# MisterBourbaki/vector-quantization-by-ml

Measured on AMD Instinct MI355X. Metric: vectors quantized/sec on [B*N,D]x[K,D] argmin; indices bit-exact vs CPU, higher is better.
Workload: dtype f32; 1 GPU; VectorQuantize dim=256 codebook_size=1024, batch [256,1024,256] per GPU, eval

## Files before the change

vector-quantization-by-ml_amd/csrc/vq_kernels.hip:

```cpp

#include <hip/hip_runtime.h>
#include <stdint.h>
#include <stdio.h>
#include <stdlib.h>
#include <string.h>

#include <initializer_list>
#include <type_traits>

#include "../../include/vq_mi355x.h"

#ifndef VQ_PART
#define VQ_PART -1
#endif
#define VQ_OWN(part) (VQ_PART < 0 || VQ_PART == (part))

typedef float f32x2 __attribute__((ext_vector_type(2)));
typedef float f32x4 __attribute__((ext_vector_type(4)));
typedef float f32x16 __attribute__((ext_vector_type(16)));

namespace {

#include "vq_common.inc"
#if VQ_OWN(0)
// ... 105 lines not shown
        return c;
    }
    static const bool no_persist = getenv("VQ_NO_PERSIST") != nullptr;
    const bool train = p.ste || p.loss_part;
    const int nsub = p.ntiles * sub_tiles(DP);
    if (whole_call && !no_persist && DP == 256 && waves == 8 && p.Q == 1 && !p.lse && !p.xt && p.vec_x && p.vec_fin && p.D % 4 == 0 &&
        (p.out || p.loss_part) &&
        !(train && getenv("VQ_NO_PERSIST_TRAIN") != nullptr) &&
        nsub >= kPersistMinSub && nsub <= kPersistMaxSub &&
        one_block_grid_x(p.M, waves) * H >= 2ll * cus) {
        c.kind = kPersist;
        c.train = train;
        c.screened = !train && metric == VQ_METRIC_EUCLID && !p.best && getenv("VQ_NO_SCREEN") == nullptr &&
                     (scr_cached ? screen_list_bytes(H, p.M) : screen_bytes(H, p.M, p.ntiles)) <= scr_room &&
                     scr_image_bytes(p.ntiles) < (1ll << 31) && (long long)H * p.M < (1ll << 31);
        c.cached = c.screened && scr_cached;
        return c;
    }
    if (DP == 512 && p.tiles_per_split >= 8 && use_pair512() &&
        (p.Q == 1 || (getenv("VQ_PAIR_NO_MULTI") == nullptr && p.Q <= PairGeo::max_stages()))) {
        c.kind = kPair;
        c.waves = 8;
    }
    return c;
}

template <int DP, int WAVES, int METRIC, int MULTI, bool LSE = false, int XT = 0, int WIDE = 0>
int launch_search_t(const SearchParams &p, int H, int splits, hipStream_t s) {
    using G = Geo<DP, WAVES>;
    const size_t lds = (size_t)(MULTI ? G::MAIN_FLOATS_M : G::MAIN_FLOATS_S) * 4 + (size_t)WAVES * p.Q * 32 * 4 +
                       ((MULTI && p.loss_part) ? (size_t)WAVES * p.Q * 64 * 4 : 0);
    if (lds > 160 * 1024) return fail(VQ_E_UNSUPPORTED, "vq_search: LDS budget exceeded (too many residual stages)");
    return launch<vq_search_mfma<DP, WAVES, METRIC, MULTI, LSE, XT, WIDE>, kBigLds>(
        dim3((unsigned)one_block_grid_x(p.M, WAVES), (unsigned)H, (unsigned)splits), dim3(WAVES * 64), lds, s, "vq_search_mfma launch", p);
}

template <int DP, int WAVES>
constexpr size_t multi_lds_bytes(int Q, bool with_loss) {
    return (size_t)Geo<DP, WAVES>::MAIN_FLOATS_M * 4 + (size_t)WAVES * Q * 32 * 4 + (with_loss ? (size_t)WAVES * Q * 64 * 4 : 0);
}

template <int DP, int WAVES>
int max_stages_t(bool with_loss) {
    int q = 1;
    while (q < 4096 && multi_lds_bytes<DP, WAVES>(q + 1, with_loss) <= 160 * 1024) ++q;
    return q;
}

template <int DP, int WAVES>
int launch_search_m(const SearchParams &p, int H, int splits, int metric, hipStream_t s) {
    return with_metric(metric, [&](auto m) {
        constexpr int ME = decltype(m)::value;
        if (p.Q > 1)
            return p.ste ? launch_search_t<DP, WAVES, ME, 2>(p, H, splits, s) : launch_search_t<DP, WAVES, ME, 1>(p, H, splits, s);
        if (p.xt == 1) return launch_search_t<DP, WAVES, ME, 0, false, 1>(p, H, splits, s);
        if (p.xt == 2) return launch_search_t<DP, WAVES, ME, 0, false, 2>(p, H, splits, s);
        if (p.lse) return launch_search_t<DP, WAVES, ME, 0, true>(p, H, splits, s);
        return launch_search_t<DP, WAVES, ME, 0>(p, H, splits, s);
    });
}

template <int METRIC, bool LSE = false, int XT = 0, int WIDE = 0, int MULTI = 0>
int launch_pair_t(const SearchParams &p, int H, int splits, hipStream_t s) {
    return launch<vq_search_pair512<METRIC, LSE, XT, WIDE, MULTI>, kBigLds>(dim3((unsigned)pair_grid_x(p.M), (unsigned)H, (unsigned)splits), dim3(512),
                                                                            PairGeo::lds_bytes(MULTI ? p.Q : 1), s, "vq_search_pair512 launch", p);
}

#if VQ_OWN(4)
int launch_pair_any(const SearchParams &p, int H, int splits, int metric, hipStream_t s) {
    return with_metric(metric, [&](auto m) {
        constexpr int ME = decltype(m)::value;
        if (p.Q > 1)
            return p.ste ? launch_pair_t<ME, false, 0, 0, 2>(p, H, splits, s) : launch_pair_t<ME, false, 0, 0, 1>(p, H, splits, s);
        if (p.xt == 1) return launch_pair_t<ME, false, 1>(p, H, splits, s);
        if (p.xt == 2) return launch_pair_t<ME, false, 2>(p, H, splits, s);
        if (p.lse) return launch_pair_t<ME, true>(p, H, splits, s);
        return launch_pair_t<ME>(p, H, splits, s);
    });
}
#endif

template <int DP>
int launch_pack_scr(const float *packed, long long pk_hs, int K, int ntiles, int H, char *img, long long img_hs, unsigned *ctrl, hipStream_t s) {
    return launch<vq_pack_scr_kernel<DP>>(dim3((unsigned)ntiles, (unsigned)H), dim3(256), 0, s, "vq_pack_scr launch", packed, pk_hs, K, ntiles, img,
                                           img_hs, ctrl);
}

template <int METRIC, bool TRAIN = false, bool SCREEN = false>
int launch_persist_t(const SearchParams &p, int H, int cus, hipStream_t s, bool scr_cached = false) {
    using G = Geo<256, 8>;
    const size_t lds = (size_t)G::MAIN_FLOATS_S * 4 + 2 * 8 * 32 * 4;
    if constexpr (SCREEN) {
        if (!scr_cached)
            if (int rc = launch_pack_scr<256>(p.packed, p.pk_hs, p.K, p.ntiles, H, (char *)p.scr, p.scr_hs, p.scr_count, s)) return rc;
    }
    if (int rc = launch<vq_search_persist<256, 8, METRIC, TRAIN, SCREEN>, kBigLds>(dim3((unsigned)persist_grid_x(p.M, H, cus), (unsigned)H, 1), dim3(512),
                                                                                   lds, s, "vq_search_persist launch", p))
        return rc;
    if constexpr (SCREEN) {
        const int flags = getenv("VQ_RESOLVE_NO_SPLIT") ? kResolveNoSplit : 0;
        return launch<vq_resolve_rows_kernel<256>, kBigLds>(dim3((unsigned)(cus > 0 ? cus : 1)), dim3(kResolveWaves * 64), resolve_lds_bytes<256>(), s,
                                                            "vq_resolve_rows launch", p, H, flags);
    }
    return 0;
}

template <int DP, int METRIC>
int launch_resident_t(const SearchParams &p, int H, int cus, hipStream_t s) {
    const size_t lds = ResGeo<DP>::lds_bytes(p.res_img_floats, p.res_nbuf);
    const long long nwb = (p.M + 31) / 32;
    long long gx = cus / H;
    if (gx < 1) gx = 1;
    if (gx > (nwb + 7) / 8) gx = (nwb + 7) / 8;
    auto go = [&](auto multibuf) {
        return launch<vq_search_resident<DP, METRIC, decltype(multibuf)::value>, kBigLds>(dim3((unsigned)gx, (unsigned)H, 1), dim3(512), lds, s,
                                                                                          "vq_search_resident launch", p);
    };
    if constexpr (DP < 128) {
        if (p.res_nbuf > 1) return go(std::true_type{});
    }
    return go(std::false_type{});
}

template <int DP>
int launch_resident_m(const SearchParams &p, int H, int cus, int metric, hipStream_t s) {
    return with_metric(metric, [&](auto m) { return launch_resident_t<DP, decltype(m)::value>(p, H, cus, s); });
}

template <int DP, int WAVES, int METRIC, int MODE>
int launch_aux_t(const AuxParams &p, int H, hipStream_t s) {
    return launch<vq_sweep_aux<DP, WAVES, METRIC, MODE>, kBigLds>(dim3((unsigned)one_block_grid_x(p.M, WAVES), (unsigned)H, 1), dim3(WAVES * 64),
                                                                  (size_t)Geo<DP, WAVES>::MAIN_FLOATS * 4, s, "vq_sweep_aux launch", p);
}

template <int DP, int WAVES>
int launch_aux_m(const AuxParams &p, int H, int metric, int mode, hipStream_t s) {
    return with_metric(metric, [&](auto m) {
        constexpr int ME = decltype(m)::value;
        return mode == kAuxSims ? launch_aux_t<DP, WAVES, ME, kAuxSims>(p, H, s) : launch_aux_t<DP, WAVES, ME, kAuxStats>(p, H, s);
    });
}

template <int DP, int METRIC>
int launch_ce_bwd_t(const CeBwdParams &p, int H, hipStream_t s) {
    const size_t stage_floats = (size_t)4 * (32 * CeGeo<DP>::GS + 96), main_floats = (size_t)Geo<DP, 4>::MAIN_FLOATS;
    return launch<vq_ce_backward<DP, METRIC>, kBigLds>(dim3((unsigned)((p.M + 127) / 128), (unsigned)H, (unsigned)CeGeo<DP>::NH), dim3(256),
                                                       4 * (main_floats > stage_floats ? main_floats : stage_floats), s, "vq_ce_backward launch", p);
}

template <int METRIC>
int launch_ce_bwd_roles_t(const CeBwdParams &p, int H, hipStream_t s) {
    return launch<vq_ce_backward_roles<METRIC>, kBigLds>(dim3((unsigned)((p.M + 32 * CeRolesGeo::NB - 1) / (32 * CeRolesGeo::NB)), (unsigned)H, 1),
                                                         dim3(512), (size_t)CeRolesGeo::LDS_F * 4, s, "vq_ce_backward_roles launch", p);
}

template <int METRIC>
int launch_ce_bwd_roles512_t(const CeBwdParams &p, int H, hipStream_t s) {
    return launch<vq_ce_backward_roles512<METRIC>, kBigLds>(dim3((unsigned)((p.M + 32 * CeRoles512Geo::NQ - 1) / (32 * CeRoles512Geo::NQ)), (unsigned)H, 1),
                                                            dim3(512), (size_t)CeRoles512Geo::LDS_F * 4, s, "vq_ce_backward_roles512 launch", p);
}

template <int DP>
int launch_ce_bwd_m(const CeBwdParams &p, int H, int metric, hipStream_t s) {
    return with_metric(metric, [&](auto m) {
        constexpr int ME = decltype(m)::value;
        if constexpr (DP == 256 || DP == 512) {
// ... 2023 lines not shown
```

vector-quantization-by-ml_amd/csrc/vq_search_persist.inc:

```
constexpr int kScrRowBytes = 1040;
constexpr int kScrTileBytes = kTileCodes * kScrRowBytes + 128;
constexpr int kScrCnOffset = kTileCodes * kScrRowBytes;
#ifndef VQ_SCR_LATE_GROUP
#define VQ_SCR_LATE_GROUP 8
#endif
constexpr int kScrLateGroup = VQ_SCR_LATE_GROUP;
inline long long scr_image_bytes(int ntiles) { return ((long long)ntiles * kScrTileBytes + 4ll * ntiles + 255) / 256 * 256; }
#include "vq_resolve_plan.h"
constexpr int kScrCtrlBytes = 16384;
constexpr int kScrTicketWord = 2, kScrLastCountsWord = 4, kScrRowTicketWord = 8;
constexpr int kScrSlotWord = kScrRowTicketWord + (int)kResolveMaxSplitRows;
static_assert(kScrSlotWord % 2 == 0 && (kScrSlotWord + 2 * (int)(kResolveMaxSplitRows * kResolveMaxSplit)) * 4 <= kScrCtrlBytes,
              "8-byte slots, inside the block");

typedef __bf16 bf16x8 __attribute__((ext_vector_type(8)));
typedef float f32x8 __attribute__((ext_vector_type(8)));

__device__ __forceinline__ void split_bf16x2(const f32x8 &v, bf16x8 &hi, bf16x8 &lo) {
    hi = __builtin_convertvector(v, bf16x8);
    const f32x8 r = v - __builtin_convertvector(hi, f32x8);
    lo = __builtin_convertvector(r, bf16x8);
}

template <int DP>
__global__ void __launch_bounds__(256) vq_pack_scr_kernel(const float *__restrict__ packed, long long pk_hs, int K, int ntiles,
                                                          char *__restrict__ img, long long img_hs, unsigned *__restrict__ ctrl) {
    static_assert(DP == 256, "the screened sweep is built for Dp = 256");
    static_assert(kScrCtrlBytes % (256 * 16) == 0, "whole rounds of 16 B per thread");
    if (blockIdx.x == 0 && blockIdx.y == 0) {
#pragma unroll
        for (int i = 0; i < kScrCtrlBytes / (256 * 16); ++i) ((uint4 *)ctrl)[i * 256 + threadIdx.x] = make_uint4(0u, 0u, 0u, 0u);
    }
    constexpr int RS = DP + 4;
    const int t = blockIdx.x, c = threadIdx.x >> 3, part = threadIdx.x & 7;
    const int k = t * kTileCodes + c;
    const float *prow = packed + (long long)blockIdx.y * pk_hs + (long long)k * RS;
    char *tile = img + (long long)blockIdx.y * img_hs + (long long)t * kScrTileBytes;
    char *dst = tile + c * kScrRowBytes;
#pragma unroll
    for (int ss = 0; ss < 2; ++ss) {
        const int s = 2 * part + ss;
#pragma unroll
        for (int h = 0; h < 2; ++h) {
            const int g = 2 * s + h;
            const f32x4 ev = *(const f32x4 *)(prow + 8 * g), od = *(const f32x4 *)(prow + 8 * g + 4);
            const f32x8 v = {ev.x, od.x, ev.y, od.y, ev.z, od.z, ev.w, od.w};
            bf16x8 hi, lo;
            split_bf16x2(v, hi, lo);
            *(bf16x8 *)(dst + 64 * s + 16 * h) = hi;
            *(bf16x8 *)(dst + 64 * s + 32 + 16 * h) = lo;
        }
    }
    if (part == 0) *(f32x4 *)(dst + 1024) = (f32x4){0.0f, 0.0f, 0.0f, 0.0f};
    float cmax = 0.0f;
    if (part == 0) {
        *(float *)(tile + kScrCnOffset + 4 * c) = prow[DP];
        cmax = (k < K) ? prow[DP + 2] : 0.0f;
    }
    __shared__ float red[kTileCodes];
    if (part == 0) red[c] = cmax;
    __syncthreads();
    if (threadIdx.x == 0) {
        float m = 0.0f;
        for (int i = 0; i < kTileCodes; ++i) m = (red[i] > m || red[i] != red[i]) ? red[i] : m;
        *(float *)(img + (long long)blockIdx.y * img_hs + (long long)ntiles * kScrTileBytes + 4 * t) = m;
    }
}

constexpr int kExChunk = 32;
constexpr int kExStageRow = kExChunk + 4;
constexpr int kExCodes = 64;
__device__ __forceinline__ float exact_chain8(float acc, const f32x4 &xa, const f32x4 &xb, const f32x4 &ce, const f32x4 &co) {
    acc = fmaf(xa.x, ce.x, acc);
    acc = fmaf(xa.y, co.x, acc);
    acc = fmaf(xa.z, ce.y, acc);
    acc = fmaf(xa.w, co.y, acc);
    acc = fmaf(xb.x, ce.z, acc);
    acc = fmaf(xb.y, co.z, acc);
    acc = fmaf(xb.z, ce.w, acc);
    acc = fmaf(xb.w, co.w, acc);
    return acc;
}
__device__ __forceinline__ float exact_dist(float acc, float xn, float cn) {
    float tt = fmaf(1.0f, xn, acc);
    tt = fmaf(cn, 1.0f, tt);
    tt = (tt < 0.0f) ? 0.0f : tt;
    return sqrtf(tt);
}
__device__ __forceinline__ bool better_euclid(bool on, float ov, int oi, bool bn, float bv, int bi) {
    if (on != bn) return on;
    if (bn) return oi < bi;
    return (ov < bv) || (ov == bv && oi < bi);
}
template <int DP>
__device__ __forceinline__ void exact_row_euclid(const float *rowbuf, float *stage, const float *pk, int kbeg, int kend, int lane,
                                                 bool &bn, float &bv, int &bi) {
    constexpr int RS = DP + 4, CD = kExChunk, SR = kExStageRow, NCH = DP / CD, NL = kExCodes / 8;
    static_assert(DP % CD == 0, "whole chunks");
    bv = __builtin_inff();
    bi = (kbeg + lane < kend) ? kbeg + lane : 0x7FFFFFFF;
    bn = false;
    const int piece = lane & 7, sub = lane >> 3;
    const float *cr = stage + lane * SR;
#pragma clang loop unroll(disable)
    for (int kb = kbeg; kb < kend; kb += kExCodes) {
        const int k = kb + lane;
        const bool ok = k < kend;
        const float *src[NL];
#pragma unroll
        for (int i = 0; i < NL; ++i) {
            const int kk = kb + sub + 8 * i;
            src[i] = pk + (long long)(kk < kend ? kk : kend - 1) * RS + 4 * piece;
        }
        f32x4 g[NL];
#pragma unroll
        for (int i = 0; i < NL; ++i) g[i] = *(const f32x4 *)(src[i]);
        const float cn = pk[(long long)(ok ? k : kend - 1) * RS + DP];
        float acc = 0.0f, xn = 0.0f;
#pragma clang loop unroll(disable)
        for (int ch = 0; ch < NCH; ++ch) {
#pragma unroll
            for (int i = 0; i < NL; ++i) *(f32x4 *)(stage + (sub + 8 * i) * SR + 4 * piece) = g[i];
            if (ch + 1 < NCH) {
#pragma unroll
                for (int i = 0; i < NL; ++i) g[i] = *(const f32x4 *)(src[i] + (ch + 1) * CD);
            }
#pragma unroll
            for (int q = 0; q < CD / 8; ++q) {
                const f32x4 ce = *(const f32x4 *)(cr + 8 * q), co = *(const f32x4 *)(cr + 8 * q + 4);
                const f32x4 xa = *(const f32x4 *)(rowbuf + ch * CD + 8 * q), xb = *(const f32x4 *)(rowbuf + ch * CD + 8 * q + 4);
                xn = fmaf(xa.x, xa.x, xn);
                xn = fmaf(xa.y, xa.y, xn);
                xn = fmaf(xa.z, xa.z, xn);
                xn = fmaf(xa.w, xa.w, xn);
                xn = fmaf(xb.x, xb.x, xn);
                xn = fmaf(xb.y, xb.y, xn);
                xn = fmaf(xb.z, xb.z, xn);
                xn = fmaf(xb.w, xb.w, xn);
                acc = exact_chain8(acc, xa, xb, ce, co);
            }
            asm volatile("s_waitcnt lgkmcnt(0)" ::: "memory");
        }
        const float s = exact_dist(acc, xn, cn);
        if (ok && !bn) {
            if (s != s) {
                bn = true;
                bv = s;
                bi = k;
// ... 181 lines not shown
            }
            bool finish = true;
            if (pl.S > 1) {
                unsigned long long *slots = (unsigned long long *)(ctrl + kScrSlotWord) + (size_t)e * kResolveMaxSplit;
                unsigned *ticket = ctrl + kScrRowTicketWord + e;
                int last = 0;
                if (lane == 0) {
                    __hip_atomic_store(slots + s, resolve_slot_pack(bn, bv, bi), __ATOMIC_RELAXED, __HIP_MEMORY_SCOPE_AGENT);
                    asm volatile("s_waitcnt vmcnt(0)" ::: "memory");
                    last = __hip_atomic_fetch_add(ticket, 1u, __ATOMIC_RELAXED, __HIP_MEMORY_SCOPE_AGENT) == pl.S - 1u ? 1 : 0;
                }
                finish = __shfl(last, 0) != 0;
                if (finish) {
                    const unsigned long long mine =
                        (unsigned)lane < pl.S ? __hip_atomic_load(slots + lane, __ATOMIC_RELAXED, __HIP_MEMORY_SCOPE_AGENT) : 0ull;
                    const unsigned lo = (unsigned)mine, hi = (unsigned)(mine >> 32);
                    bn = (__shfl(lo, 0) & 0x80000000u) != 0u;
                    bv = __uint_as_float(__shfl(hi, 0));
                    bi = (int)(__shfl(lo, 0) & 0x7FFFFFFFu);
                    for (unsigned i = 1; i < pl.S; ++i) {
                        const unsigned olo = __shfl(lo, (int)i), ohi = __shfl(hi, (int)i);
                        const bool on = (olo & 0x80000000u) != 0u;
                        const float ov = __uint_as_float(ohi);
                        const int oi = (int)(olo & 0x7FFFFFFFu);
                        if (better_euclid(on, ov, oi, bn, bv, bi)) {
                            bn = on;
                            bv = ov;
                            bi = oi;
                        }
                    }
                    if (lane == 0) __hip_atomic_store(ticket, 0u, __ATOMIC_RELAXED, __HIP_MEMORY_SCOPE_AGENT);
                }
            }
            if (finish) {
                if (lane == 0) p.idx[(long long)head * p.idx_hs + row * p.idx_rs] = bi;
                const int dl = 4 * lane;
                if (p.out && dl < p.D)
                    *(f32x4 *)(p.out + (long long)head * p.out_hs + row * p.out_rs + dl) =
                        *(const f32x4 *)(p.cb + (long long)head * p.cb_hs + (long long)bi * p.D + dl);
            }
        }
    }
    unsigned bfirst, bstride;
    resolve_wave_batches(pl, grid, wg, (unsigned)wave, bfirst, bstride);
    for (unsigned b = bfirst; b < pl.nbatch; b += bstride) rescore_batch<DP>(p, cap, b * kRsEntries, n1, stage, xstage, lane);
    if (tid == 0) {
        if (exit_ticket == grid - 1u) {
            __hip_atomic_store(ctrl + kScrLastCountsWord, listed0, __ATOMIC_RELAXED, __HIP_MEMORY_SCOPE_AGENT);
            __hip_atomic_store(ctrl + kScrLastCountsWord + 1, listed1, __ATOMIC_RELAXED, __HIP_MEMORY_SCOPE_AGENT);
            __hip_atomic_store(ctrl + 0, 0u, __ATOMIC_RELAXED, __HIP_MEMORY_SCOPE_AGENT);
            __hip_atomic_store(ctrl + 1, 0u, __ATOMIC_RELAXED, __HIP_MEMORY_SCOPE_AGENT);
            __hip_atomic_store(ctrl + kScrTicketWord, 0u, __ATOMIC_RELAXED, __HIP_MEMORY_SCOPE_AGENT);
        }
    }
}

#ifdef VQ_EXP_SCREEN_COUNT
__device__ unsigned long long g_scr_rows[3];
#endif

template <int DP, int WAVES, int METRIC, bool TRAIN = false, bool SCREEN = false>
__global__ void __launch_bounds__(WAVES * 64, 2) vq_search_persist(const SearchParams p) {
    static_assert(!SCREEN || (DP == 256 && METRIC == VQ_METRIC_EUCLID && !TRAIN), "screened sweep: Dp = 256, Euclid, inference");
    using G = Geo<DP, WAVES>;
    constexpr int RS = G::RS, RS4 = G::RS4, CH = G::CH, XS = G::XS, NS = G::NS, SUB = G::SUB;
    constexpr bool EUCLID = (METRIC == VQ_METRIC_EUCLID);
    static_assert(G::NCH4 == 1 || DP == 512, "one float4 per lane covers a row");

    extern __shared__ __attribute__((aligned(16))) float smem[];
    f32x4 *tile4 = (f32x4 *)smem;
    lds_f32x4 *tile4_lds = (lds_f32x4 *)smem;
    static_assert(G::SEP_STAGE, "rows are staged behind the tile buffers (one 8-wave workgroup per CU)");
    int *sidx = (int *)(smem + G::MAIN_FLOATS_S);

    const int tid = threadIdx.x;
    const int lane = tid & 63;
    const int wave = __builtin_amdgcn_readfirstlane(tid >> 6);
    const int c = lane & 31, h = lane >> 5;
    const int head = blockIdx.y;
    const float *xh = p.x + (long long)head * p.x_hs;
    const float *pk = p.packed + (long long)head * p.pk_hs;
    const float *cbh = p.cb + (long long)head * p.cb_hs;
    const float *scrh = SCREEN ? (const float *)((const char *)p.scr + head * p.scr_hs) : nullptr;
    float scr_mcn = 0.0f;
    if constexpr (SCREEN) {
        const float *tmax = (const float *)((const char *)scrh + (long long)p.ntiles * kScrTileBytes);
        for (int i = lane; i < p.ntiles; i += 64) {
            const float v = tmax[i];
            scr_mcn = (v > scr_mcn || v != v) ? v : scr_mcn;
        }
#pragma unroll
        for (int o = 32; o > 0; o >>= 1) {
            const float v = __shfl_xor(scr_mcn, o);
            scr_mcn = (v > scr_mcn || v != v) ? v : scr_mcn;
        }
        scr_mcn = __uint_as_float(__builtin_amdgcn_readfirstlane(__float_as_uint(scr_mcn)));
    }
    float *outh = p.out ? p.out + (long long)head * p.out_hs : nullptr;
    const float INF = __builtin_inff();
    const int nblk = (int)((p.M + 32 * WAVES - 1) / (32 * WAVES));
    const int dl = 4 * lane;
    const bool dok = dl < p.D;
    const bool scr_late = SCREEN && p.scr_stagger != 0 && wave >= 4;

    int cp_rows = 0, cp_next = 0;
    long long cp_row0 = 0;
    const int *cp_idx = sidx;
    int cp_pend = -1;
    f32x4 cp_v = {0.0f, 0.0f, 0.0f, 0.0f};
    f32x4 cp_x = {0.0f, 0.0f, 0.0f, 0.0f};
    float cp_e = 0.0f;
    int cp_iv = 0;
    auto train_quant = [&](const f32x4 &cv, const f32x4 &xv) -> f32x4 {
        const f32x4 diff = cv - xv;
        cp_e = fmaf(diff.x, diff.x, cp_e);
        cp_e = fmaf(diff.y, diff.y, cp_e);
        cp_e = fmaf(diff.z, diff.z, cp_e);
        cp_e = fmaf(diff.w, diff.w, cp_e);
        return p.ste ? xv + diff : cv;
    };
    auto copy_step = [&]() {
        if (cp_pend >= 0) {
            if (dok) {
                f32x4 o = cp_v;
                if constexpr (TRAIN) o = train_quant(cp_v, cp_x);
                if (p.out) __builtin_nontemporal_store(o, (f32x4 *)(outh + (cp_row0 + cp_pend) * p.out_rs + dl));
            }
            cp_pend = -1;
        }
        if (cp_next < cp_rows) {
            const int i = __builtin_amdgcn_readfirstlane(cp_iv);
            if (dok) {
                cp_v = *(const f32x4 *)(cbh + (long long)i * p.D + dl);
                if constexpr (TRAIN) cp_x = *(const f32x4 *)(xh + (cp_row0 + cp_next) * p.x_rs + dl);
            }
            cp_pend = cp_next;
            ++cp_next;
            if (cp_next < cp_rows) cp_iv = cp_idx[cp_next];
        }
    };

    auto stage = [&](int tile, int buf) {
        if constexpr (SCREEN) {
            static_assert(kScrTileBytes <= G::BUF_F4 * 16, "a bf16x3 tile fits the fp32 tile's buffer");
#pragma unroll
            for (int i2 = 0; i2 < (G::TILE_CHUNKS + WAVES - 1) / WAVES; ++i2) {
                const int ck = i2 * WAVES + wave;
                if (ck < (kScrTileBytes + 1023) / 1024)
                    lds_dma16(scrh, p.scr_bytes, lane * 16, tile * kScrTileBytes + ck * 1024, tile4_lds + buf * G::BUF_F4 + ck * 64);
            }
        } else {
            stage_tile<G, WAVES>(pk, p.pk_bytes, tile, tile4_lds + buf * G::BUF_F4, wave, lane);
        }
    };
#define PSTAMP(j) do { if (it < 8) STAMP(4 * it + (j)); } while (0)
#define SSTAMP(j) do { if (it == 2 && u >= 12 && u < 18) STAMP(32 + 4 * (u - 12) + (j)); } while (0)
    int it = 0;
    long long row0 = 0;
    STAMP_RT(60);
    for (int blk = blockIdx.x; blk < nblk; blk += gridDim.x, ++it) {
        row0 = ((long long)blk * WAVES + wave) * 32;
        PSTAMP(0);
        stage(0, 0);
        __builtin_amdgcn_s_setprio(2);
        float xf[NS];
        bf16x8 xhf[SCREEN ? DP / 16 : 1], xlf[SCREEN ? DP / 16 : 1];
        float xn0 = 0.0f;
        {
            float *xs = smem + G::NBUF * G::BUF_F4 * 4 + wave * (32 * XS);
            constexpr int NCHUNK = DP / CH;
            constexpr int LPL = CH / 8;
            f32x4 v[2][LPL];
            auto load_chunk = [&](int ch, f32x4 (&dst)[LPL]) {
#pragma unroll
                for (int i2 = 0; i2 < LPL; ++i2) {
                    const int f = i2 * 64 + lane;
                    const int r = f / (CH / 4), c4 = f % (CH / 4);
                    long long grow = row0 + r;
                    if (grow >= p.M) grow = p.M - 1;
                    const int d0 = ch * CH + c4 * 4;
                    f32x4 t = {0.0f, 0.0f, 0.0f, 0.0f};
                    if (d0 < p.D) t = __builtin_nontemporal_load((const f32x4 *)(xh + grow * p.x_rs + d0));
                    dst[i2] = t;
                }
            };
            load_chunk(0, v[0]);
#pragma unroll
            for (int ch = 0; ch < NCHUNK; ++ch) {
                if (ch + 1 < NCHUNK) load_chunk(ch + 1, v[(ch + 1) & 1]);
#pragma unroll
                for (int i2 = 0; i2 < LPL; ++i2) {
                    const int f = i2 * 64 + lane;
                    const int r = f / (CH / 4), c4 = f % (CH / 4);
                    *(f32x4 *)(xs + r * XS + c4 * 4) = v[ch & 1][i2];
                }
                asm volatile("s_waitcnt lgkmcnt(0)" ::: "memory");
                const float *rp = xs + c * XS;
                f32x4 plo, phi;
#pragma unroll
                for (int j = 0; j < CH / 8; ++j) {
                    const f32x4 lo = *(const f32x4 *)(rp + 8 * j);
                    const f32x4 hi = *(const f32x4 *)(rp + 8 * j + 4);
                    if (EUCLID) {
                        xn0 = fmaf(lo.x, lo.x, xn0);
                        xn0 = fmaf(lo.y, lo.y, xn0);
                        xn0 = fmaf(lo.z, lo.z, xn0);
                        xn0 = fmaf(lo.w, lo.w, xn0);
                        xn0 = fmaf(hi.x, hi.x, xn0);
                        xn0 = fmaf(hi.y, hi.y, xn0);
                        xn0 = fmaf(hi.z, hi.z, xn0);
                        xn0 = fmaf(hi.w, hi.w, xn0);
                        asm volatile("" : "+v"(xn0));
                    }
                    if constexpr (SCREEN) {
                        if (j & 1) {
                            const f32x8 v8 = h ? (f32x8){lo.x, lo.y, lo.z, lo.w, hi.x, hi.y, hi.z, hi.w}
                                               : (f32x8){plo.x, plo.y, plo.z, plo.w, phi.x, phi.y, phi.z, phi.w};
                            const int sg = ch * (CH / 16) + (j >> 1);
                            split_bf16x2(v8, xhf[sg], xlf[sg]);
                        } else {
                            plo = lo;
                            phi = hi;
                        }
                        continue;
                    }
                    const f32x4 m = h ? hi : lo;
                    const auto xy = __builtin_amdgcn_permlane32_swap(__float_as_uint(m.x), __float_as_uint(m.y), false, false);
                    const auto zw = __builtin_amdgcn_permlane32_swap(__float_as_uint(m.z), __float_as_uint(m.w), false, false);
                    const int sb = ch * (CH / 2) + 4 * j;
                    xf[sb + 0] = __uint_as_float(xy[0]);
                    xf[sb + 1] = __uint_as_float(zw[0]);
                    xf[sb + 2] = __uint_as_float(xy[1]);
                    xf[sb + 3] = __uint_as_float(zw[1]);
                }
                asm volatile("s_waitcnt lgkmcnt(0)" ::: "memory");
            }
        }
        __builtin_amdgcn_s_setprio(0);
        const long long row = row0 + c;
        const bool row_ok = row < p.M;
        const float b_aug = EUCLID ? (h ? 1.0f : xn0) : 1.0f;

        const unsigned cb_flag = codebook_flag(pk, p.pk_bytes);
        LaneBest lb = lane_best_start<METRIC>(SCREEN ? INF : sweep_start_value<METRIC>(cb_flag));
        float scr_b2 = INF, scr_b3 = INF;
        int scr_i2 = 0;
        auto epilogue = [&](const f32x16 &v, int u) {
            if constexpr (SCREEN) {
                const float o1 = lb.best_t, o2 = scr_b2;
                float b1 = o1, b2 = o2;
#define VQ_SCR_STEP(r) "v_med3_f32 %2, %1, %2, %" #r "\n\tv_med3_f32 %1, %0, %1, %" #r "\n\tv_min_f32 %0, %0, %" #r "\n\t"
                asm(VQ_SCR_STEP(3) VQ_SCR_STEP(4) VQ_SCR_STEP(5) VQ_SCR_STEP(6) VQ_SCR_STEP(7) VQ_SCR_STEP(8) VQ_SCR_STEP(9)
                    VQ_SCR_STEP(10) VQ_SCR_STEP(11) VQ_SCR_STEP(12) VQ_SCR_STEP(13) VQ_SCR_STEP(14) VQ_SCR_STEP(15) VQ_SCR_STEP(16)
                    VQ_SCR_STEP(17) VQ_SCR_STEP(18)
                    : "+v"(b1), "+v"(b2), "+v"(scr_b3)
                    : "v"(v[0]), "v"(v[1]), "v"(v[2]), "v"(v[3]), "v"(v[4]), "v"(v[5]), "v"(v[6]), "v"(v[7]), "v"(v[8]), "v"(v[9]),
                      "v"(v[10]), "v"(v[11]), "v"(v[12]), "v"(v[13]), "v"(v[14]), "v"(v[15]));
#undef VQ_SCR_STEP
                const bool nb1 = b1 < o1;
                if (nb1 || b2 < o2) {
                    int off1 = 0, off2 = 0;
#pragma unroll
                    for (int r = 15; r >= 0; --r) off1 = (v[r] == b1) ? (r & 3) + 8 * (r >> 2) : off1;
#pragma unroll
                    for (int r = 15; r >= 0; --r) {
                        const int o = (r & 3) + 8 * (r >> 2);
                        off2 = (v[r] == b2 && !(nb1 && o == off1)) ? o : off2;
                    }
                    const int base = u * kTileCodes + 4 * h;
                    const int i1 = lb.pend_u;
                    scr_i2 = (nb1 && b2 == o1) ? i1 : base + off2;
                    if (nb1) lb.pend_u = base + off1;
                    lb.best_t = b1;
                    scr_b2 = b2;
                }
            } else {
                tile_epilogue<METRIC, DP, false>(v, u, h, p.K, lb);
            }
        };

        const int t1 = p.ntiles;
        auto run_sub_scr = [&](f32x16 &acc, f32x16 &prev, int u, bool have_prev) {
            constexpr int NGS = DP / 16, PF = 3;
            static_assert(kScrLateGroup > 3 && kScrLateGroup < NGS, "the late epilogue sits inside the last range of groups");
            SSTAMP(0);
            const int cur = u & 1;
            const char *tb = (const char *)(tile4 + cur * G::BUF_F4);
            const char *ta = tb + c * kScrRowBytes + 16 * h;
            bf16x8 ah[NGS], al[NGS];
            {
                const f32x4 *cn4 = (const f32x4 *)(tb + kScrCnOffset);
#pragma unroll
                for (int q = 0; q < 4; ++q) {
                    const f32x4 cv = cn4[2 * q + h];
                    acc[4 * q + 0] = cv.x; acc[4 * q + 1] = cv.y; acc[4 * q + 2] = cv.z; acc[4 * q + 3] = cv.w;
                }
            }
#pragma unroll
            for (int g = 0; g < PF; ++g) {
                ah[g] = *(const bf16x8 *)(ta + 64 * g);
                al[g] = *(const bf16x8 *)(ta + 64 * g + 32);
            }
            copy_step();
            auto groups = [&](auto g0c, auto g1c) {
                constexpr int G0 = decltype(g0c)::value, G1 = decltype(g1c)::value;
#pragma unroll
                for (int g = G0; g < G1; ++g) {
                    if (g + PF < NGS) {
                        ah[g + PF] = *(const bf16x8 *)(ta + 64 * (g + PF));
                        al[g + PF] = *(const bf16x8 *)(ta + 64 * (g + PF) + 32);
                    }
                    acc = __builtin_amdgcn_mfma_f32_32x32x16_bf16(ah[g], xhf[g], acc, 0, 0, 0);
                    acc = __builtin_amdgcn_mfma_f32_32x32x16_bf16(al[g], xhf[g], acc, 0, 0, 0);
                    acc = __builtin_amdgcn_mfma_f32_32x32x16_bf16(ah[g], xlf[g], acc, 0, 0, 0);
                    __builtin_amdgcn_sched_barrier(0);
                }
            };
            groups(IntC<0>{}, IntC<1>{});
            if (have_prev && !scr_late) {
                SSTAMP(1);
                epilogue(prev, u - 1);
                SSTAMP(2);
            }
            __builtin_amdgcn_sched_barrier(0);
            groups(IntC<1>{}, IntC<3>{});
            if (u + 1 < t1) stage(u + 1, cur ^ 1);
            __builtin_amdgcn_sched_barrier(0);
            groups(IntC<3>{}, IntC<kScrLateGroup>{});
            if (have_prev && scr_late) {
                SSTAMP(1);
                epilogue(prev, u - 1);
                SSTAMP(2);
            }
            __builtin_amdgcn_sched_barrier(0);
            groups(IntC<kScrLateGroup>{}, IntC<NGS>{});
            SSTAMP(3);
            __syncthreads();
        };
        auto run_sub = [&](f32x16 &acc, f32x16 &prev, int u, bool have_prev) {
            if constexpr (SCREEN) {
                run_sub_scr(acc, prev, u, have_prev);
                return;
            }
            const int t = u / SUB, st = u % SUB;
            const int cur = t & 1;
            const f32x4 *tb = tile4 + cur * G::BUF_F4 + st * (kTileCodes * RS4);
            constexpr int NG = DP / 8;
            constexpr int G1 = NG >= 2 ? 1 : NG, G2 = NG >= 4 ? 3 : NG;
            const f32x4 *ta = tb + c * RS4 + h;
            f32x4 a[NG];
            acc = (f32x16){0};
            const float a_aug = EUCLID ? ((const float *)tb)[c * RS + DP + 1 - h] : 0.0f;
            mfma_prefetch<DP>(a, ta);
            copy_step();
            mfma_range<DP, 0, G1>(acc, a, ta, xf);
            if (have_prev) epilogue(prev, u - 1);
            __builtin_amdgcn_sched_barrier(0);
            mfma_range<DP, G1, G2>(acc, a, ta, xf);
            if (st == 0 && t + 1 < t1) stage(t + 1, cur ^ 1);
            __builtin_amdgcn_sched_barrier(0);
            mfma_range<DP, G2, NG>(acc, a, ta, xf);
            if (EUCLID) {
                acc = __builtin_amdgcn_mfma_f32_32x32x2f32(a_aug, b_aug, acc, 0, 0, 0);
            }
            if (st == SUB - 1) __syncthreads();
        };

        PSTAMP(1);
        __syncthreads();
        {
            f32x16 acc0, acc1;
            int u = 0;
            const int u1 = t1 * SUB;
            bool have_prev = false;
            for (; u + 1 < u1; u += 2) {
                run_sub(acc0, acc1, u, have_prev);
                run_sub(acc1, acc0, u + 1, true);
                have_prev = true;
            }
            if (u < u1) {
                run_sub(acc0, acc1, u, have_prev);
                epilogue(acc0, u);
            } else if (have_prev) {
                epilogue(acc1, u - 1);
            }
        }
        while (cp_next < cp_rows || cp_pend >= 0) copy_step();
        PSTAMP(2);

        float best_s;
        int best_i;
        long long cand = 0;
        bool has_cand = false;
        if constexpr (SCREEN) {
            const float l1 = lb.best_t, l2 = scr_b2;
            const int li1 = lb.pend_u, li2 = scr_i2;
            best_i = li1 < p.K ? li1 : p.K - 1;
            float b1 = l1;
            const float ob1 = __shfl_xor(l1, 32), ob2 = __shfl_xor(l2, 32), ob3 = __shfl_xor(scr_b3, 32);
            const int oi = __shfl_xor(best_i, 32);
            const float b2 = fminf(fmaxf(l1, ob1), fminf(l2, ob2));
            if (ob1 < b1 || (ob1 == b1 && oi < best_i)) {
                b1 = ob1;
                best_i = oi;
            }
            const float nx = sqrtf(xn0), nc = sqrtf(scr_mcn);
            const float delta = 2.5e-4f * (2.0f * nx * nc) + 1e-4f * scr_mcn + 3e-7f * xn0 + 0x1p-110f * (1.0f + nx + nc);
            const float w = 0x1p-20f * (__builtin_fabsf(b1) + xn0 + delta);
            const bool eligible = cb_flag == 0u && xn0 <= 0x1p100f && scr_mcn <= 0x1p100f && (b1 + xn0 > 2.0f * delta);
            const bool certain = eligible && (b2 - b1 > 2.0f * delta + w);
            best_s = 0.0f;
            const float thr = b1 + 2.0f * delta + w;
            const bool complete = eligible && scr_b3 > thr && ob3 > thr;
            const unsigned rescore = (unsigned)__ballot(row_ok && !certain && complete);
            const unsigned todo = (unsigned)__ballot(row_ok && !certain && !complete);
#ifdef VQ_EXP_SCREEN_COUNT
            const unsigned rows_here = (unsigned)__ballot(row_ok);
            if (lane == 0) {
                atomicAdd(&g_scr_rows[0], (unsigned long long)__builtin_popcount(todo));
                atomicAdd(&g_scr_rows[1], (unsigned long long)__builtin_popcount(rows_here));
                atomicAdd(&g_scr_rows[2], (unsigned long long)__builtin_popcount(rescore));
            }
#endif
            if (rescore != 0u) {
                const unsigned my = ((l1 <= thr) ? (unsigned)li1 : 0xFFFFu) | (((l2 <= thr) ? (unsigned)li2 : 0xFFFFu) << 16);
                const unsigned other = (unsigned)__shfl_xor((int)my, 32);
                unsigned at = 0u;
                if (lane == 0) at = atomicAdd(p.scr_count + 1, (unsigned)__builtin_popcount(rescore));
                at = __builtin_amdgcn_readfirstlane(at);
                if (h == 0 && ((rescore >> c) & 1u)) {
                    const unsigned cap = (unsigned)((long long)gridDim.y * p.M);
                    p.scr_list[cap - 1u - (at + __builtin_popcount(rescore & ((1u << c) - 1u)))] = (unsigned)((long long)head * p.M + row);
                    cand = (long long)(((unsigned long long)other << 32) | my);
                    has_cand = true;
                }
            }
            if (todo != 0u) {
                unsigned at = 0u;
                if (lane == 0) at = atomicAdd(p.scr_count, (unsigned)__builtin_popcount(todo));
                at = __builtin_amdgcn_readfirstlane(at);
                if (h == 0 && ((todo >> c) & 1u))
                    p.scr_list[at + __builtin_popcount(todo & ((1u << c) - 1u))] = (unsigned)((long long)head * p.M + row);
            }
        } else {
        resolve_best<METRIC>(lb, h, p.K, best_s, best_i);
        {
            const float os = __shfl_xor(best_s, 32);
            const int oi = __shfl_xor(best_i, 32);
            const bool take = EUCLID ? (os < best_s || (os == best_s && oi < best_i))
                                     : (os > best_s || (os == best_s && oi < best_i));
            if (take) {
                best_s = os;
                best_i = oi;
            }
        }
        if (const unsigned todo = nonfinite_rows(best_s, row_ok); __builtin_expect(todo != 0u, 0)) {
            float *rowbuf = smem + G::NBUF * G::BUF_F4 * 4 + wave * (32 * XS);
            auto fill_row = [&](int rr) -> float {
#pragma clang loop unroll(disable)
                for (int d = lane; d < DP; d += 64) rowbuf[d] = (d < p.D) ? xh[(row0 + rr) * p.x_rs + d] : 0.0f;
                return 0.0f;
            };
            auto acc_init = [&](int, int) -> float { return 0.0f; };
            repair_nonfinite_rows<METRIC, DP>(todo, rowbuf, pk, 0, p.K, lane, fill_row, acc_init, best_s, best_i);
        }
        }
        PSTAMP(3);
        if (h == 0 && row_ok) {
            const long long o = (long long)head * p.idx_hs + row * p.idx_rs;
            p.idx[o] = has_cand ? cand : (long long)best_i;
            if (p.best) p.best[o] = best_s;
        }
        int *mine = sidx + ((it & 1) * WAVES + wave) * 32;
        mine[c] = best_i;
        cp_rows = (p.M - row0 >= 32) ? 32 : (p.M - row0 > 0 ? (int)(p.M - row0) : 0);
        cp_row0 = row0;
        cp_idx = mine;
        cp_next = 0;
        cp_pend = -1;
        if (cp_rows > 0) cp_iv = mine[0];
    }

    __builtin_amdgcn_s_setprio(2);
    constexpr int RB = 4;
    for (int rr0 = 0; rr0 < cp_rows; rr0 += RB) {
        f32x4 o[RB], xv[RB];
#pragma unroll
        for (int k = 0; k < RB; ++k) {
            const int rr = (rr0 + k < cp_rows) ? rr0 + k : cp_rows - 1;
            const int i = cp_idx[rr];
            o[k] = dok ? *(const f32x4 *)(cbh + (long long)i * p.D + dl) : (f32x4){0.0f, 0.0f, 0.0f, 0.0f};
            if constexpr (TRAIN) xv[k] = dok ? *(const f32x4 *)(xh + (cp_row0 + rr) * p.x_rs + dl) : (f32x4){0.0f, 0.0f, 0.0f, 0.0f};
// ... 25 lines not shown
```

Before: 653.2 million vectors/s.

## Screen with scaled fp16 single-half codebook instead of bf16 hi/lo split

Stores the screening codebook as one power-of-two-scaled fp16 value per element instead of bf16 hi+lo pairs. This halves the screening tile bytes and cuts the MFMA count per group from three to two. A new absmax pre-pass picks the global scale exponent, and the pack kernel records per-tile quantization error, L1 and flag bounds. The screening margin is recomputed from these bounds so exact fallback stays bit-exact. In exchange it adds an extra launch, a serial loop over tiles in every pack block, and possibly looser margins that send more rows to rescoring.

```diff
diff --git a/vector-quantization-by-ml_amd/csrc/vq_kernels.hip b/vector-quantization-by-ml_amd/csrc/vq_kernels.hip
--- a/vector-quantization-by-ml_amd/csrc/vq_kernels.hip
+++ b/vector-quantization-by-ml_amd/csrc/vq_kernels.hip
@@ -211,6 +211,9 @@
 
 template <int DP>
 int launch_pack_scr(const float *packed, long long pk_hs, int K, int ntiles, int H, char *img, long long img_hs, unsigned *ctrl, hipStream_t s) {
+    if (int rc = launch<vq_scr_absmax_kernel<DP>>(dim3((unsigned)ntiles, (unsigned)H), dim3(256), 0, s, "vq_scr_absmax launch", packed, pk_hs, ntiles,
+                                                  img, img_hs))
+        return rc;
     return launch<vq_pack_scr_kernel<DP>>(dim3((unsigned)ntiles, (unsigned)H), dim3(256), 0, s, "vq_pack_scr launch", packed, pk_hs, K, ntiles, img,
                                            img_hs, ctrl);
 }
diff --git a/vector-quantization-by-ml_amd/csrc/vq_search_persist.inc b/vector-quantization-by-ml_amd/csrc/vq_search_persist.inc
--- a/vector-quantization-by-ml_amd/csrc/vq_search_persist.inc
+++ b/vector-quantization-by-ml_amd/csrc/vq_search_persist.inc
@@ -1,11 +1,19 @@
-constexpr int kScrRowBytes = 1040;
+constexpr int kScrRowBytes = 528;
 constexpr int kScrTileBytes = kTileCodes * kScrRowBytes + 128;
 constexpr int kScrCnOffset = kTileCodes * kScrRowBytes;
+constexpr int kScrChunks = (kScrTileBytes + 1023) / 1024;
+constexpr int kScrTailMcn = 0, kScrTailEc = 1, kScrTailL1 = 2, kScrTailFlag = 3, kScrTailAbs = 4, kScrTailExp = 5;
+constexpr int kScrMaxExp = 62;
+constexpr int kScrTileRoom = kTileCodes * 1040 + 128;
+static_assert(kScrChunks * 1024 + 4 * kScrTailExp + 8 <= kScrTileRoom + 4, "tiles, over-copy and tail fit the room of one tile");
 #ifndef VQ_SCR_LATE_GROUP
 #define VQ_SCR_LATE_GROUP 8
 #endif
 constexpr int kScrLateGroup = VQ_SCR_LATE_GROUP;
-inline long long scr_image_bytes(int ntiles) { return ((long long)ntiles * kScrTileBytes + 4ll * ntiles + 255) / 256 * 256; }
+#ifndef VQ_SCR_PF
+#define VQ_SCR_PF 3
+#endif
+inline long long scr_image_bytes(int ntiles) { return ((long long)ntiles * kScrTileRoom + 4ll * ntiles + 255) / 256 * 256; }
 #include "vq_resolve_plan.h"
 constexpr int kScrCtrlBytes = 16384;
 constexpr int kScrTicketWord = 2, kScrLastCountsWord = 4, kScrRowTicketWord = 8;
@@ -13,13 +21,37 @@
 static_assert(kScrSlotWord % 2 == 0 && (kScrSlotWord + 2 * (int)(kResolveMaxSplitRows * kResolveMaxSplit)) * 4 <= kScrCtrlBytes,
               "8-byte slots, inside the block");
 
-typedef __bf16 bf16x8 __attribute__((ext_vector_type(8)));
+typedef _Float16 f16x8 __attribute__((ext_vector_type(8)));
 typedef float f32x8 __attribute__((ext_vector_type(8)));
 
-__device__ __forceinline__ void split_bf16x2(const f32x8 &v, bf16x8 &hi, bf16x8 &lo) {
-    hi = __builtin_convertvector(v, bf16x8);
+__device__ __forceinline__ void split_f16x2(const f32x8 &v, f16x8 &hi, f16x8 &lo) {
+    hi = __builtin_convertvector(v, f16x8);
     const f32x8 r = v - __builtin_convertvector(hi, f32x8);
-    lo = __builtin_convertvector(r, bf16x8);
+    lo = __builtin_convertvector(r, f16x8);
+}
+__device__ __forceinline__ float scr_pow2(int e) { return __uint_as_float((unsigned)(e + 127) << 23); }
+
+template <int DP>
+__global__ void __launch_bounds__(256) vq_scr_absmax_kernel(const float *__restrict__ packed, long long pk_hs, int ntiles,
+                                                            char *__restrict__ img, long long img_hs) {
+    constexpr int RS = DP + 4;
+    static_assert(DP == 256, "8 threads per code, 32 floats each");
+    const int t = blockIdx.x, c = threadIdx.x >> 3, part = threadIdx.x & 7;
+    const float *prow = packed + (long long)blockIdx.y * pk_hs + (long long)(t * kTileCodes + c) * RS + 32 * part;
+    float m = 0.0f;
+#pragma unroll
+    for (int i = 0; i < 8; ++i) {
+        const f32x4 v = *(const f32x4 *)(prow + 4 * i);
+        m = fmaxf(m, fmaxf(fmaxf(__builtin_fabsf(v.x), __builtin_fabsf(v.y)), fmaxf(__builtin_fabsf(v.z), __builtin_fabsf(v.w))));
+    }
+#pragma unroll
+    for (int o = 32; o > 0; o >>= 1) m = fmaxf(m, __shfl_xor(m, o));
+    __shared__ float red[4];
+    if ((threadIdx.x & 63) == 0) red[threadIdx.x >> 6] = m;
+    __syncthreads();
+    if (threadIdx.x == 0)
+        ((float *)(img + (long long)blockIdx.y * img_hs + (long long)ntiles * kScrTileBytes))[kScrTailAbs * ntiles + t] =
+            fmaxf(fmaxf(red[0], red[1]), fmaxf(red[2], red[3]));
 }
 
 template <int DP>
@@ -35,8 +67,25 @@
     const int t = blockIdx.x, c = threadIdx.x >> 3, part = threadIdx.x & 7;
     const int k = t * kTileCodes + c;
     const float *prow = packed + (long long)blockIdx.y * pk_hs + (long long)k * RS;
-    char *tile = img + (long long)blockIdx.y * img_hs + (long long)t * kScrTileBytes;
+    char *himg = img + (long long)blockIdx.y * img_hs;
+    char *tile = himg + (long long)t * kScrTileBytes;
+    float *tail = (float *)(himg + (long long)ntiles * kScrTileBytes);
     char *dst = tile + c * kScrRowBytes;
+    float hmax = 0.0f;
+    for (int i = 0; i < ntiles; ++i) hmax = fmaxf(hmax, tail[kScrTailAbs * ntiles + i]);
+    int e_c = 0, e_x = 0;
+    unsigned flag = 0u;
+    if (hmax != 0.0f) {
+        const int lg = (int)((__float_as_uint(hmax) >> 23) & 0xFFu) - 127;
+        e_c = 13 - lg;
+        e_x = e_c - 5;
+        if (e_c > kScrMaxExp || e_c < -kScrMaxExp || e_x > kScrMaxExp || e_x < -kScrMaxExp) {
+            e_c = e_x = 0;
+            flag = 1u;
+        }
+    }
+    const float s_c = scr_pow2(e_c), sg = scr_pow2(e_c + e_x);
+    float d2 = 0.0f, l1 = 0.0f;
 #pragma unroll
     for (int ss = 0; ss < 2; ++ss) {
         const int s = 2 * part + ss;
@@ -44,26 +93,57 @@
         for (int h = 0; h < 2; ++h) {
             const int g = 2 * s + h;
             const f32x4 ev = *(const f32x4 *)(prow + 8 * g), od = *(const f32x4 *)(prow + 8 * g + 4);
-            const f32x8 v = {ev.x, od.x, ev.y, od.y, ev.z, od.z, ev.w, od.w};
-            bf16x8 hi, lo;
-            split_bf16x2(v, hi, lo);
-            *(bf16x8 *)(dst + 64 * s + 16 * h) = hi;
-            *(bf16x8 *)(dst + 64 * s + 32 + 16 * h) = lo;
-        }
-    }
-    if (part == 0) *(f32x4 *)(dst + 1024) = (f32x4){0.0f, 0.0f, 0.0f, 0.0f};
-    float cmax = 0.0f;
+            const f32x8 v = (f32x8){ev.x, od.x, ev.y, od.y, ev.z, od.z, ev.w, od.w} * s_c;
+            f16x8 ct = __builtin_convertvector(v, f16x8);
+            f32x8 cf = __builtin_convertvector(ct, f32x8);
+#pragma unroll
+            for (int e = 0; e < 8; ++e) {
+                if (__builtin_fabsf(cf[e]) < 0x1p-14f) {
+                    ct[e] = (_Float16)0.0f;
+                    cf[e] = 0.0f;
+                }
+                const float d = v[e] - cf[e];
+                d2 = fmaf(d, d, d2);
+                l1 += __builtin_fabsf(cf[e]);
+            }
+            *(f16x8 *)(dst + 32 * s + 16 * h) = ct;
+        }
+    }
+#pragma unroll
+    for (int o = 1; o < 8; o <<= 1) {
+        d2 += __shfl_xor(d2, o);
+        l1 += __shfl_xor(l1, o);
+    }
+    __shared__ float red_cn[kTileCodes], red_ec[kTileCodes], red_l1[kTileCodes];
+    __shared__ unsigned red_fl[kTileCodes];
     if (part == 0) {
-        *(float *)(tile + kScrCnOffset + 4 * c) = prow[DP];
-        cmax = (k < K) ? prow[DP + 2] : 0.0f;
-    }
-    __shared__ float red[kTileCodes];
-    if (part == 0) red[c] = cmax;
+        *(f32x4 *)(dst + 512) = (f32x4){0.0f, 0.0f, 0.0f, 0.0f};
+        const float cn = prow[DP];
+        const float cs = cn * sg;
+        *(float *)(tile + kScrCnOffset + 4 * c) = cs;
+        const bool real = k < K;
+        red_cn[c] = real ? prow[DP + 2] : 0.0f;
+        red_ec[c] = real ? sqrtf(d2) * (1.0f + 0x1p-10f) : 0.0f;
+        red_l1[c] = real ? l1 * (1.0f + 0x1p-10f) : 0.0f;
+        red_fl[c] = (real && cn < __builtin_inff() && !(cs == 0.0f ? cn == 0.0f : (cs >= 0x1p-126f && cs < __builtin_inff()))) ? 1u : 0u;
+    }
     __syncthreads();
     if (threadIdx.x == 0) {
-        float m = 0.0f;
-        for (int i = 0; i < kTileCodes; ++i) m = (red[i] > m || red[i] != red[i]) ? red[i] : m;
-        *(float *)(img + (long long)blockIdx.y * img_hs + (long long)ntiles * kScrTileBytes + 4 * t) = m;
+        float m = 0.0f, ec = 0.0f, ml1 = 0.0f;
+        for (int i = 0; i < kTileCodes; ++i) {
+            m = (red_cn[i] > m || red_cn[i] != red_cn[i]) ? red_cn[i] : m;
+            ec = (red_ec[i] > ec || red_ec[i] != red_ec[i]) ? red_ec[i] : ec;
+            ml1 = (red_l1[i] > ml1 || red_l1[i] != red_l1[i]) ? red_l1[i] : ml1;
+            flag |= red_fl[i];
+        }
+        tail[kScrTailMcn * ntiles + t] = m;
+        tail[kScrTailEc * ntiles + t] = ec;
+        tail[kScrTailL1 * ntiles + t] = ml1;
+        ((unsigned *)tail)[kScrTailFlag * ntiles + t] = flag;
+        if (t == 0) {
+            ((int *)tail)[kScrTailExp * ntiles] = e_c;
+            ((int *)tail)[kScrTailExp * ntiles + 1] = e_x;
+        }
     }
 }
 
@@ -411,19 +491,40 @@
     const float *pk = p.packed + (long long)head * p.pk_hs;
     const float *cbh = p.cb + (long long)head * p.cb_hs;
     const float *scrh = SCREEN ? (const float *)((const char *)p.scr + head * p.scr_hs) : nullptr;
-    float scr_mcn = 0.0f;
+    float scr_mcn = 0.0f, scr_ecs = 0.0f, scr_abs = 0.0f, scr_sx = 1.0f, scr_isg = 1.0f;
+    unsigned scr_flag = 0u;
     if constexpr (SCREEN) {
-        const float *tmax = (const float *)((const char *)scrh + (long long)p.ntiles * kScrTileBytes);
+        const float *tail = (const float *)((const char *)scrh + (long long)p.ntiles * kScrTileBytes);
+        float ec = 0.0f, l1 = 0.0f;
+        auto nanmax = [](float a, float v) { return (v > a || v != v) ? v : a; };
         for (int i = lane; i < p.ntiles; i += 64) {
-            const float v = tmax[i];
-            scr_mcn = (v > scr_mcn || v != v) ? v : scr_mcn;
+            scr_mcn = nanmax(scr_mcn, tail[kScrTailMcn * p.ntiles + i]);
+            ec = nanmax(ec, tail[kScrTailEc * p.ntiles + i]);
+            l1 = nanmax(l1, tail[kScrTailL1 * p.ntiles + i]);
+            scr_flag |= ((const unsigned *)tail)[kScrTailFlag * p.ntiles + i];
         }
 #pragma unroll
         for (int o = 32; o > 0; o >>= 1) {
-            const float v = __shfl_xor(scr_mcn, o);
-            scr_mcn = (v > scr_mcn || v != v) ? v : scr_mcn;
-        }
+            scr_mcn = nanmax(scr_mcn, __shfl_xor(scr_mcn, o));
+            ec = nanmax(ec, __shfl_xor(ec, o));
+            l1 = nanmax(l1, __shfl_xor(l1, o));
+            scr_flag |= (unsigned)__shfl_xor((int)scr_flag, o);
+        }
+        int e_c = ((const int *)tail)[kScrTailExp * p.ntiles], e_x = ((const int *)tail)[kScrTailExp * p.ntiles + 1];
+        if (e_c > kScrMaxExp || e_c < -kScrMaxExp || e_x > kScrMaxExp || e_x < -kScrMaxExp) {
+            e_c = e_x = 0;
+            scr_flag = 1u;
+        }
+        scr_sx = scr_pow2(e_x);
+        scr_isg = scr_pow2(-(e_c + e_x));
+        scr_ecs = ec * scr_pow2(-e_c);
+        scr_abs = (0x1p-13f * l1 + 0x1p-116f) * scr_isg + 0x1p-140f;
         scr_mcn = __uint_as_float(__builtin_amdgcn_readfirstlane(__float_as_uint(scr_mcn)));
+        scr_ecs = __uint_as_float(__builtin_amdgcn_readfirstlane(__float_as_uint(scr_ecs)));
+        scr_abs = __uint_as_float(__builtin_amdgcn_readfirstlane(__float_as_uint(scr_abs)));
+        scr_sx = __uint_as_float(__builtin_amdgcn_readfirstlane(__float_as_uint(scr_sx)));
+        scr_isg = __uint_as_float(__builtin_amdgcn_readfirstlane(__float_as_uint(scr_isg)));
+        scr_flag = __builtin_amdgcn_readfirstlane(scr_flag);
     }
     float *outh = p.out ? p.out + (long long)head * p.out_hs : nullptr;
     const float INF = __builtin_inff();
@@ -471,11 +572,11 @@
 
     auto stage = [&](int tile, int buf) {
         if constexpr (SCREEN) {
-            static_assert(kScrTileBytes <= G::BUF_F4 * 16, "a bf16x3 tile fits the fp32 tile's buffer");
-#pragma unroll
-            for (int i2 = 0; i2 < (G::TILE_CHUNKS + WAVES - 1) / WAVES; ++i2) {
+            static_assert(kScrChunks * 1024 <= G::BUF_F4 * 16, "an fp16 tile fits the fp32 tile's buffer");
+#pragma unroll
+            for (int i2 = 0; i2 < (kScrChunks + WAVES - 1) / WAVES; ++i2) {
                 const int ck = i2 * WAVES + wave;
-                if (ck < (kScrTileBytes + 1023) / 1024)
+                if (ck < kScrChunks)
                     lds_dma16(scrh, p.scr_bytes, lane * 16, tile * kScrTileBytes + ck * 1024, tile4_lds + buf * G::BUF_F4 + ck * 64);
             }
         } else {
@@ -493,7 +594,7 @@
         stage(0, 0);
         __builtin_amdgcn_s_setprio(2);
         float xf[NS];
-        bf16x8 xhf[SCREEN ? DP / 16 : 1], xlf[SCREEN ? DP / 16 : 1];
+        f16x8 xhf[SCREEN ? DP / 16 : 1], xlf[SCREEN ? DP / 16 : 1];
         float xn0 = 0.0f;
         {
             float *xs = smem + G::NBUF * G::BUF_F4 * 4 + wave * (32 * XS);
@@ -546,7 +647,7 @@
                             const f32x8 v8 = h ? (f32x8){lo.x, lo.y, lo.z, lo.w, hi.x, hi.y, hi.z, hi.w}
                                                : (f32x8){plo.x, plo.y, plo.z, plo.w, phi.x, phi.y, phi.z, phi.w};
                             const int sg = ch * (CH / 16) + (j >> 1);
-                            split_bf16x2(v8, xhf[sg], xlf[sg]);
+                            split_f16x2(v8 * scr_sx, xhf[sg], xlf[sg]);
                         } else {
                             plo = lo;
                             phi = hi;
@@ -610,13 +711,13 @@
 
         const int t1 = p.ntiles;
         auto run_sub_scr = [&](f32x16 &acc, f32x16 &prev, int u, bool have_prev) {
-            constexpr int NGS = DP / 16, PF = 3;
+            constexpr int NGS = DP / 16, PF = VQ_SCR_PF;
             static_assert(kScrLateGroup > 3 && kScrLateGroup < NGS, "the late epilogue sits inside the last range of groups");
             SSTAMP(0);
             const int cur = u & 1;
             const char *tb = (const char *)(tile4 + cur * G::BUF_F4);
             const char *ta = tb + c * kScrRowBytes + 16 * h;
-            bf16x8 ah[NGS], al[NGS];
+            f16x8 ah[NGS];
             {
                 const f32x4 *cn4 = (const f32x4 *)(tb + kScrCnOffset);
 #pragma unroll
@@ -626,22 +727,15 @@
                 }
             }
 #pragma unroll
-            for (int g = 0; g < PF; ++g) {
-                ah[g] = *(const bf16x8 *)(ta + 64 * g);
-                al[g] = *(const bf16x8 *)(ta + 64 * g + 32);
-            }
+            for (int g = 0; g < PF; ++g) ah[g] = *(const f16x8 *)(ta + 32 * g);
             copy_step();
             auto groups = [&](auto g0c, auto g1c) {
                 constexpr int G0 = decltype(g0c)::value, G1 = decltype(g1c)::value;
 #pragma unroll
                 for (int g = G0; g < G1; ++g) {
-                    if (g + PF < NGS) {
-                        ah[g + PF] = *(const bf16x8 *)(ta + 64 * (g + PF));
-                        al[g + PF] = *(const bf16x8 *)(ta + 64 * (g + PF) + 32);
-                    }
-                    acc = __builtin_amdgcn_mfma_f32_32x32x16_bf16(ah[g], xhf[g], acc, 0, 0, 0);
-                    acc = __builtin_amdgcn_mfma_f32_32x32x16_bf16(al[g], xhf[g], acc, 0, 0, 0);
-                    acc = __builtin_amdgcn_mfma_f32_32x32x16_bf16(ah[g], xlf[g], acc, 0, 0, 0);
+                    if (g + PF < NGS) ah[g + PF] = *(const f16x8 *)(ta + 32 * (g + PF));
+                    acc = __builtin_amdgcn_mfma_f32_32x32x16_f16(ah[g], xhf[g], acc, 0, 0, 0);
+                    acc = __builtin_amdgcn_mfma_f32_32x32x16_f16(ah[g], xlf[g], acc, 0, 0, 0);
                     __builtin_amdgcn_sched_barrier(0);
                 }
             };
@@ -722,7 +816,8 @@
         long long cand = 0;
         bool has_cand = false;
         if constexpr (SCREEN) {
-            const float l1 = lb.best_t, l2 = scr_b2;
+            const float l1 = lb.best_t * scr_isg, l2 = scr_b2 * scr_isg;
+            scr_b3 *= scr_isg;
             const int li1 = lb.pend_u, li2 = scr_i2;
             best_i = li1 < p.K ? li1 : p.K - 1;
             float b1 = l1;
@@ -734,9 +829,10 @@
                 best_i = oi;
             }
             const float nx = sqrtf(xn0), nc = sqrtf(scr_mcn);
-            const float delta = 2.5e-4f * (2.0f * nx * nc) + 1e-4f * scr_mcn + 3e-7f * xn0 + 0x1p-110f * (1.0f + nx + nc);
+            const float delta = 1.1f * (1.0001f * scr_ecs * nx + 4.63e-5f * (2.0f * nx * nc) + 3.07e-5f * scr_mcn + 1.21e-7f * xn0 + scr_abs);
             const float w = 0x1p-20f * (__builtin_fabsf(b1) + xn0 + delta);
-            const bool eligible = cb_flag == 0u && xn0 <= 0x1p100f && scr_mcn <= 0x1p100f && (b1 + xn0 > 2.0f * delta);
+            const bool eligible = cb_flag == 0u && scr_flag == 0u && xn0 * scr_sx * scr_sx <= 0x1p30f && scr_mcn <= 0x1p100f &&
+                                  (b1 + xn0 > 2.0f * delta);
             const bool certain = eligible && (b2 - b1 > 2.0f * delta + w);
             best_s = 0.0f;
             const float thr = b1 + 2.0f * delta + w;
```

New measurement: 794.4 million vectors/s, median of 6. 21.6% higher.
